# sandialabs/implicit-sph

Hardware: AMD Instinct MI355X
Metric: pressure-Poisson solves/sec (3D TGV, 1M particles per GPU, GMRES(50)+block-Jacobi ILU(0), tol 1e-8) (higher is better)
Workload: dtype f64; 1 GPU; 3D Taylor-Green vortex, 100^3 particles per GPU, Wendland cut=2h (BASELINE configs[1]), state after one Lagrangian step (mode=advect); rows_per_gpu=1000000, global_rows=1000000, nnz_per_gpu=103845090, solver=FGMRES(50) DGKS tol 1e-8, right prec, precond=bjacobi-ilu0, atom_order=lexicographic, library_row_order=bricks, parallelism=domain bricks 1x1x1, RCCL halo + all-reduce, restarts=1, converged=1

## Files before the change

### implicit-sph_amd/csrc/ilu.hpp

```cpp
#pragma once
#include <cfloat>
#include <cmath>
#include "core.hpp"
#include "sell.hpp"

struct isph_ilu {
  int n = 0, B = 0, nblocks = 0, wmax = 0;
  isph::DevBuf<long long> frp;
  isph::DevBuf<int> fcol, flen, fdiag, err;
  isph::DevBuf<double> fval;
  isph::DevBuf<double> sv;
  int value_bits = 64;
  isph::DevBuf<float> svf;
  isph::DevBuf<unsigned short> sc;
  isph::DevBuf<unsigned char> si;
  isph::DevBuf<unsigned short> sperm;
  isph::DevBuf<int> fdst;
  isph::DevBuf<int> blkinfo;
  isph::DevBuf<int> llev;
  isph::DevBuf<double> dinv;
  isph::DevBuf<long long> boff;
  isph::DevBuf<long long> sboff;
  bool exact = false;
  long long stream_entries = 0;
  bool compact = false;
  const long long *stream_off() const { return exact ? sboff.p : boff.p; }
  isph::DevBuf<unsigned char> flev;
  long long stream_chunks = 0;
  long long total = 0;
  int fill = 0;
  int capf = 0, slack = 0;
  isph::DevBuf<int> bptr;
  const int *blocks() const { return bptr.p; }
};

namespace isph {

__device__ __forceinline__ void ilu_block_rows(const int *__restrict__ bptr, int b, int B, int n, int &blo, int &bhi) {
  if (bptr) { blo = bptr[b]; bhi = bptr[b + 1]; }
  else { blo = b * B; bhi = min(blo + B, n); }
}

constexpr int kExtChunk = 8;
constexpr int kExtAhead = 8;

template <bool REFILL = false>
__global__ __launch_bounds__(1024) void k_ilu_extract(int n, int B, const int *__restrict__ rowlen,
                                                      const long long *__restrict__ slice_off,
                                                      const int *__restrict__ scol, const double *__restrict__ sval,
                                                      long long *__restrict__ frp, int *__restrict__ fcol,
                                                      double *__restrict__ fval, int *__restrict__ flen,
                                                      int *__restrict__ fdiag, int *__restrict__ err, int b0,
                                                      const long long *__restrict__ base_off,
                                                      const int *__restrict__ bptr, int *__restrict__ badrow = nullptr) {
  __shared__ int wsum[16];
  extern __shared__ double ext_lds[];
  const int nwv = blockDim.x >> 6;
  double (*stage_val)[64][kExtChunk] = reinterpret_cast<double (*)[64][kExtChunk]>(ext_lds);
  long long (*stage_start)[64] = reinterpret_cast<long long (*)[64]>(ext_lds + (size_t)nwv * 64 * kExtChunk);
  int (*stage_col)[64][kExtChunk] = reinterpret_cast<int (*)[64][kExtChunk]>(ext_lds + (size_t)nwv * 64 * (kExtChunk + 1));
  int (*stage_cnt)[64] = reinterpret_cast<int (*)[64]>(reinterpret_cast<int *>(ext_lds + (size_t)nwv * 64 * (kExtChunk + 1)) +
                                                       (size_t)nwv * 64 * kExtChunk);
  const int b = blockIdx.x + b0;
  int blo, bhi;
// ... 578 lines not shown
            sc[idx] = (unsigned short)flags;
            sv[idx] = 0.0;
          }
        }
        if (rinfo & 1) {
          const unsigned need = (unsigned)((rinfo >> 1) & 7);
          for (int c = lane; c < rT; c += 64) si[rch0 + c] = (unsigned char)((c == rT - 1 ? 1u : 0u) | (need << 1));
          const int first = (rinfo >> 8) & 127, nun = 64 - first;
          for (int x = lane; x < rT * nun; x += 64) {
            const int c = x / nun, ln = first + x - c * nun;
            const long long idx = (rch0 + c) * 64 + ln;
            sc[idx] = 0;
            sv[idx] = 0.0;
          }
        }
      };
      int cja = colreq(0), cjb;
      for (int src = 0; src < 64; src += 2) {
        cjb = colreq(src + 1);
        emit(src, cja);
        cja = colreq(src + 2);
        emit(src + 1, cjb);
      }
    }
    used += s_nch;
    __syncthreads();
  }
}

constexpr int kFacPrefetch = 4;
constexpr int kFacPrefetchWide = 8;
constexpr int kIluWaves = 8;

template <int WAVES, bool WIDE>
__global__ __launch_bounds__(WAVES * 64, WIDE ? 1 : 8) void k_ilu_factor(int n, int B, int W, const long long *__restrict__ frp,
                                                           const int *__restrict__ fcol, double *__restrict__ fval,
                                                           const int *__restrict__ flen,
                                                           const int *__restrict__ fdiag, const int *__restrict__ fdst,
                                                           const int *__restrict__ llev, double *__restrict__ sv,
                                                           double *__restrict__ dinv, const long long *__restrict__ boff,
                                                           int capf, int slack, int b0, const int *__restrict__ err,
                                                           const int *__restrict__ bptr) {
  extern __shared__ double lds_f[];
  double *diag = lds_f;
  double *wval = diag + B;
  long long *rpL = reinterpret_cast<long long *>(wval + WAVES * W);
  int *wcol = reinterpret_cast<int *>(rpL + B);
  int *lenL = wcol + WAVES * W;
  int *dgL = lenL + B;
  int *lstart = dgL + B;
  int *lcnt = lstart + B + 2;
  int *levs = lcnt + B + 1;
  unsigned short *order = reinterpret_cast<unsigned short *>(levs + B);
  unsigned short *pos = order + B;
  __shared__ int s_nlev, s_err;
  if (threadIdx.x == 0) s_err = err != nullptr ? *err : 0;
  __syncthreads();
  if (s_err & (1 | 16 | 32)) return;
  const int bid = blockIdx.x + b0;
  int blo, bhi;
  ilu_block_rows(bptr, bid, B, n, blo, bhi);
  const int m = bhi - blo;
  const int wave = threadIdx.x >> 6, lane = threadIdx.x & 63;
  double *svb = sv + ilu_base_chunk(boff, bid, capf, slack) * 64;
  if (threadIdx.x == 0) s_nlev = 0;
  for (int t = threadIdx.x; t <= B; t += blockDim.x) lcnt[t] = 0;
  for (int t = threadIdx.x; t < WAVES * B; t += blockDim.x) pos[t] = 0;
  __syncthreads();
  for (int t = threadIdx.x; t < m; t += blockDim.x) {
    rpL[t] = frp[blo + t];
    lenL[t] = flen[blo + t];
    dgL[t] = fdiag[blo + t];
    const int l = llev[blo + t];
    levs[t] = l;
    atomicAdd(&lcnt[l], 1);
    atomicMax(&s_nlev, l + 1);
  }
  __syncthreads();
  if (threadIdx.x == 0) {
    int run = 0;
    for (int l = 0; l < s_nlev; ++l) { lstart[l] = run; run += lcnt[l]; }
    lstart[s_nlev] = run;
  }
  __syncthreads();
  for (int t = threadIdx.x; t < m; t += blockDim.x) {
    const int l = levs[t];
    int rk = 0;
    for (int q = 0; q < t; ++q) rk += (levs[q] == l);
    order[lstart[l] + rk] = (unsigned short)t;
  }
  __syncthreads();
  double *mv = wval + wave * W;
  int *mc = wcol + wave * W;
  unsigned short *mp = pos + wave * B;
  const int nlev = s_nlev;
  const long long rp_block = (long long)(((unsigned long long)(unsigned)__builtin_amdgcn_readfirstlane((int)(rpL[0] >> 32)) << 32) |
                                         (unsigned)__builtin_amdgcn_readfirstlane((int)rpL[0]));
// ... 374 lines not shown
      if (hipGetLastError() != hipSuccess) rc = fail("ILU(k) symbolic fill failed", __FILE__, __LINE__);
    }
    if (rc != ISPH_SUCCESS) { nrp.release(); ncol.release(); ndiag.release(); nlev.release(); nval.release(); break; }
    F->frp.release(); F->fcol.release(); F->fdiag.release(); F->flev.release(); F->fval.release(); F->flen.release();
    F->frp = nrp; F->fcol = ncol; F->fdiag = ndiag; F->flev = nlev; F->fval = nval;
    F->flen = nlen;
    nlen = DevBuf<int>();
    rc = nlen.reserve(n1);
    F->total = total;
    F->wmax = wmax;
  }
  nlen.release(); inoff.release(); blktot.release(); meta.release();
  if (!ctx->pattern_hold || rc != ISPH_SUCCESS) F->flev.release();
  return rc;
}

inline long long &ilu_exact_stream_bytes() {
  static long long v = 4LL << 30;
  return v;
}
inline bool ilu_wants_exact_stream(const isph_ilu *F) {
  const long long rule_chunks = kCapFactor * (F->total >> 6) + (long long)(kPadChunks + 2 * F->B) * (F->nblocks + 1) + kPadChunks;
  return rule_chunks * 64 * 10 > ilu_exact_stream_bytes();
}
inline int ilu_size_stream(isph_ilu *F) {
  const long long entries = F->exact ? F->stream_entries : F->total;
  F->stream_chunks = F->capf * (entries >> 6) + (long long)(kPadChunks + F->slack) * (F->nblocks + 1) + kPadChunks;
  int r = F->sv.reserve((size_t)F->stream_chunks * 64);
  if (r == ISPH_SUCCESS) r = F->sc.reserve((size_t)F->stream_chunks * 64);
  if (r == ISPH_SUCCESS) r = F->si.reserve((size_t)F->stream_chunks + 64);
  return r;
}

inline int ilu_begin(isph_ctx *ctx, const Sell &S, int block_size, bool sgs, int fill, isph_ilu **out, bool defer_factor_arrays = false,
                     int nblocks_tab = 0, const int *host_bptr = nullptr) {
  ISPH_REQUIRE(block_size >= 64 && block_size <= 1024 && block_size % 64 == 0,
               "block-Jacobi ILU block size must be a multiple of 64 in [64,1024]");
  ISPH_REQUIRE(fill >= 0 && fill <= 8 && !(sgs && fill), "level of fill must be in [0,8]");
  ISPH_REQUIRE(nblocks_tab == 0 || host_bptr, "a table of subdomains without its offsets");
  isph_ilu *F = new isph_ilu();
  F->n = S.nrow; F->B = block_size; F->wmax = S.wmax; F->fill = fill;
  F->nblocks = nblocks_tab > 0 ? nblocks_tab : (S.nrow + block_size - 1) / block_size;
  if (nblocks_tab > 0) {
    if (F->bptr.reserve((size_t)nblocks_tab + 1) != ISPH_SUCCESS ||
        hipMemcpyAsync(F->bptr.p, host_bptr, sizeof(int) * ((size_t)nblocks_tab + 1), hipMemcpyHostToDevice, ctx->stream) != hipSuccess ||
        hipStreamSynchronize(ctx->stream) != hipSuccess) {
      ilu_destroy(F);
      return fail("copy of the subdomain table failed", __FILE__, __LINE__);
    }
  }
  F->total = S.stored + (nblocks_tab > 0 ? 64LL * nblocks_tab : 0);
  const size_t stored = (size_t)(F->total > 0 ? F->total : 1), n1 = (size_t)(S.nrow > 0 ? S.nrow : 1);
  F->capf = kCapFactor; F->slack = 2 * block_size;
  int rc = defer_factor_arrays ? ISPH_SUCCESS : F->fcol.reserve(stored);
  if (rc == ISPH_SUCCESS && !defer_factor_arrays) rc = F->fval.reserve(stored);
  if (rc == ISPH_SUCCESS) rc = F->frp.reserve(n1);
  if (rc == ISPH_SUCCESS) rc = F->flen.reserve(n1);
  if (rc == ISPH_SUCCESS) rc = F->fdiag.reserve(n1);
  if (rc == ISPH_SUCCESS) rc = F->dinv.reserve(n1);
  if (rc == ISPH_SUCCESS) rc = F->llev.reserve(n1);
  if (rc == ISPH_SUCCESS) rc = F->err.reserve(1);
  if (rc == ISPH_SUCCESS) rc = F->boff.reserve((size_t)F->nblocks + 1);
  if (rc == ISPH_SUCCESS) rc = F->blkinfo.reserve((size_t)4 * (F->nblocks > 0 ? F->nblocks : 1));
  if (rc == ISPH_SUCCESS) rc = F->sperm.reserve((size_t)2 * block_size * (F->nblocks > 0 ? F->nblocks : 1));
  if (rc == ISPH_SUCCESS && hipMemsetAsync(F->err.p, 0, sizeof(int), ctx->stream) != hipSuccess)
    rc = fail("memset failed", __FILE__, __LINE__);
  if (rc == ISPH_SUCCESS && S.nrow > 0) {
    const size_t lds_e = (size_t)(block_size / 64) * 64 * ((kExtChunk + 1) * 8 + (kExtChunk + 1) * 4);
    const size_t lds_s = sizeof(int) * (14 * (size_t)block_size + 10) + sizeof(long long) * (size_t)block_size;
    if (hipFuncSetAttribute(reinterpret_cast<const void *>(k_ilu_extract<false>), hipFuncAttributeMaxDynamicSharedMemorySize,
                            (int)lds_e) != hipSuccess ||
        hipFuncSetAttribute(reinterpret_cast<const void *>(k_ilu_schedule<true>), hipFuncAttributeMaxDynamicSharedMemorySize,
                            (int)lds_s) != hipSuccess ||
        hipFuncSetAttribute(reinterpret_cast<const void *>(k_ilu_schedule<false>), hipFuncAttributeMaxDynamicSharedMemorySize,
// ... 13 lines not shown
  return size_stream ? ilu_size_stream(F) : ISPH_SUCCESS;
}

inline void ilu_launch_extract(isph_ctx *ctx, isph_ilu *F, const Sell &S, int b0, int nb, hipStream_t st = nullptr) {
  const size_t lds_e = (size_t)(F->B / 64) * 64 * ((kExtChunk + 1) * 8 + (kExtChunk + 1) * 4);
  ProfScope prof(ctx, PROF_ILU_EXTRACT, st);
  hipLaunchKernelGGL(k_ilu_extract<false>, dim3(nb), dim3(F->B), lds_e, st ? st : ctx->stream, S.nrow, F->B, (const int *)S.rowlen.p,
                     (const long long *)S.slice_off.p, (const int *)S.col.p, (const double *)S.val.p, F->frp.p, F->fcol.p,
                     F->fval.p, F->flen.p, F->fdiag.p, F->err.p, b0, F->compact ? (const long long *)F->boff.p : (const long long *)nullptr,
                     F->blocks(), (int *)nullptr);
}

inline void ilu_launch_schedule(isph_ctx *ctx, isph_ilu *F, const Sell &S, int b0, int nb, bool sgs, hipStream_t st = nullptr,
                                bool count_only = false) {
  const size_t Bz = (size_t)F->B;
  const size_t lds_s = sizeof(int) * (14 * Bz + 10) + sizeof(long long) * Bz;
  ProfScope prof(ctx, PROF_ILU_SCHEDULE, st);
  if (F->wmax <= 129)
    hipLaunchKernelGGL(k_ilu_schedule<true>, dim3(nb), dim3(F->B), lds_s, st ? st : ctx->stream, S.nrow, F->B, F->stream_off(), F->frp.p, F->fcol.p,
                       F->flen.p, F->fdiag.p, F->sv.p, F->sc.p, F->si.p, F->sperm.p, F->fdst.p, F->blkinfo.p, F->llev.p, F->capf,
                       F->slack, F->err.p, sgs ? (const double *)F->fval.p : (const double *)nullptr,
                       sgs ? (const double *)F->dinv.p : (const double *)nullptr, b0, count_only ? 1 : 0, F->blocks());
  else
    hipLaunchKernelGGL(k_ilu_schedule<false>, dim3(nb), dim3(F->B), lds_s, st ? st : ctx->stream, S.nrow, F->B, F->stream_off(), F->frp.p, F->fcol.p,
                       F->flen.p, F->fdiag.p, F->sv.p, F->sc.p, F->si.p, F->sperm.p, F->fdst.p, F->blkinfo.p, F->llev.p, F->capf,
                       F->slack, F->err.p, sgs ? (const double *)F->fval.p : (const double *)nullptr,
                       sgs ? (const double *)F->dinv.p : (const double *)nullptr, b0, count_only ? 1 : 0, F->blocks());
}

inline int ilu_launch_factor(isph_ctx *ctx, isph_ilu *F, const Sell &S, int b0, int nb, const int *err_dev, hipStream_t st_in = nullptr) {
  hipStream_t st = st_in ? st_in : ctx->stream;
  const size_t Bz = (size_t)F->B;
  const int W = ((F->wmax + 63) / 64) * 64;
  const size_t lds_f = 8 * Bz + (size_t)kIluWaves * W * 12 + 8 * Bz + 4 * (5 * Bz + 4) + 2 * Bz + 2 * (size_t)kIluWaves * Bz + 16;
  ISPH_REQUIRE(lds_f <= 160 * 1024, "ILU factor kernel needs too much LDS for this row width");
  const bool wide = F->wmax > 128;
  const void *fk = wide ? reinterpret_cast<const void *>(k_ilu_factor<kIluWaves, true>)
                        : reinterpret_cast<const void *>(k_ilu_factor<kIluWaves, false>);
  ISPH_CHECK_HIP(hipFuncSetAttribute(fk, hipFuncAttributeMaxDynamicSharedMemorySize, (int)lds_f));
  ProfScope prof(ctx, PROF_ILU_FACTOR, st_in);
  if (wide)
    hipLaunchKernelGGL((k_ilu_factor<kIluWaves, true>), dim3(nb), dim3(kIluWaves * 64), lds_f, st, S.nrow, F->B, W,
                       F->frp.p, F->fcol.p, F->fval.p, F->flen.p, F->fdiag.p, F->fdst.p, F->llev.p, F->sv.p, F->dinv.p, F->stream_off(),
                       F->capf, F->slack, b0, err_dev, F->blocks());
  else
    hipLaunchKernelGGL((k_ilu_factor<kIluWaves, false>), dim3(nb), dim3(kIluWaves * 64), lds_f, st, S.nrow, F->B, W,
                       F->frp.p, F->fcol.p, F->fval.p, F->flen.p, F->fdiag.p, F->fdst.p, F->llev.p, F->sv.p, F->dinv.p, F->stream_off(),
                       F->capf, F->slack, b0, err_dev, F->blocks());
  ISPH_CHECK_HIP(hipGetLastError());
  return ISPH_SUCCESS;
}

inline int ilu_schedule_and_factor(isph_ctx *ctx, isph_ilu *F, const Sell &S, bool sgs) {
  int rc = ISPH_SUCCESS;
  if (sgs)
    hipLaunchKernelGGL(k_sgs_pivots, dim3((S.nrow + kBlock - 1) / kBlock), dim3(kBlock), 0, ctx->stream, S.nrow, F->frp.p,
                       F->fval.p, F->fdiag.p, F->dinv.p);
  if (F->exact) {
    rc = F->sboff.reserve((size_t)F->nblocks + 1);
    if (rc == ISPH_SUCCESS) {
      ilu_launch_schedule(ctx, F, S, 0, F->nblocks, sgs, nullptr, true);
      hipLaunchKernelGGL(k_ilu_exact_offsets, dim3(1), dim3(1024), 0, ctx->stream, F->nblocks, (const int *)F->blkinfo.p, F->sboff.p);
      long long total = 0;
      if (hipMemcpyAsync(&total, F->sboff.p + F->nblocks, sizeof(long long), hipMemcpyDeviceToHost, ctx->stream) != hipSuccess)
        rc = fail("copy failed", __FILE__, __LINE__);
      if (rc == ISPH_SUCCESS) rc = ilu_check_err(ctx, F, "ILU extract/schedule (counting pass) failed");
// ... 462 lines not shown
```

### implicit-sph_amd/csrc/isph_capi.hip

```cpp
#include <algorithm>
#include <numeric>

#include "assemble.hpp"
#include "operators.hpp"
#include "block_helmholtz.hpp"
#include "core.hpp"
#include "ilu.hpp"
#include "krylov.hpp"
#include "sell.hpp"
#include "solver.hpp"
#include "chebyshev.hpp"
#include "amg.hpp"
#include "schwarz.hpp"
#include "prec.hpp"
#include "gcrodr.hpp"
#include "ingress.hpp"

namespace isph {
thread_local std::string g_last_error;

int sell_finalize_offsets(isph_ctx *ctx, Sell &S) {
  hipLaunchKernelGGL(k_exclusive_scan_ll, dim3(1), dim3(1024), 0, ctx->stream, S.nslices, S.slice_off.p, S.slice_off.p);
  std::vector<long long> so((size_t)S.nslices + 1, 0);
  ISPH_CHECK_HIP(hipMemcpyAsync(so.data(), S.slice_off.p, sizeof(long long) * so.size(), hipMemcpyDeviceToHost, ctx->stream));
// ... 1112 lines not shown
  return type && parse_prec_type(type, &s) ? (int)s.kind : -1;
}

int isph_prec_value_bits(const isph_prec *M) {
  if (const Cheb *C = prec_cheb(M)) return C->value_bits;
  if (const isph_amg *G = prec_amg(M)) return G->cheb ? G->cheb_value_bits : 0;
  if (const isph_ilu *F = prec_ilu(M)) return F->value_bits == 32 ? 32 : 0;
  return 0;
}

int isph_prec_cycle_bits(const isph_prec *M) {
  const isph_amg *G = prec_amg(M);
  return (G && G->cheb && G->cycle_bits == 32) ? 32 : 64;
}

int isph_prec_create(isph_ctx *ctx, const isph_mat *A, const char *type, int block_size, isph_prec **Mout) {
  ISPH_REQUIRE(ctx && A && type && Mout, "NULL argument");
  return prec_create_named(ctx, A, type, block_size, Mout);
}

int isph_prec_refactor(isph_ctx *ctx, isph_prec *M, const isph_mat *A) {
  ISPH_REQUIRE(ctx && M && A, "NULL argument");
  return prec_refactor(ctx, M, A);
}

int isph_prec_apply(isph_ctx *ctx, const isph_prec *M, const double *r, double *z, int on_device) {
  ISPH_REQUIRE(ctx && M && r && z, "NULL argument");
  return prec_apply_operands(ctx, M, r, z, on_device);
}

int isph_prec_multi_path(isph_ctx *ctx, const isph_prec *M, int nvec) {
  if (!ctx || !M) return 0;
  return prec_multi_shared(M, nvec) ? 1 : 0;
}

int isph_prec_apply_multi(isph_ctx *ctx, const isph_prec *M, int nvec, const double *r, double *z, int lda, int on_device) {
  ISPH_REQUIRE(ctx && M && r && z, "NULL argument");
  ISPH_REQUIRE(nvec >= 1, "isph_prec_apply_multi: nvec must be at least 1");
  ISPH_REQUIRE(lda >= M->n, "isph_prec_apply_multi: lda must be at least the number of rows");
  return prec_apply_multi_operands(ctx, M, nvec, r, z, lda, on_device);
}

int isph_prec_export_ilu(isph_ctx *ctx, const isph_prec *M, int *rowptr, int *colidx, double *val) {
  ISPH_REQUIRE(ctx && prec_ilu(M), "not an ILU preconditioner");
  return ilu_export(ctx, M->ilu, rowptr, colidx, val);
}

int isph_prec_info(isph_ctx *ctx, const isph_prec *M, long long info[4]) {
  ISPH_REQUIRE(ctx && M && info, "NULL argument");
  info[0] = info[1] = info[2] = info[3] = 0;
  const isph_ilu *F = prec_ilu(M);
  if (!F) return ISPH_SUCCESS;
  std::vector<int> bi((size_t)4 * F->nblocks);
  ISPH_CHECK_HIP(hipMemcpyAsync(bi.data(), F->blkinfo.p, sizeof(int) * bi.size(), hipMemcpyDeviceToHost, ctx->stream));
  ISPH_CHECK_HIP(hipStreamSynchronize(ctx->stream));
  long long used = 0;
  for (size_t b = 0; b < (size_t)F->nblocks; ++b) used += bi[4 * b] + bi[4 * b + 1];
  info[0] = ilu_nnz(F); info[1] = used; info[2] = F->stream_chunks; info[3] = F->nblocks;
  return ISPH_SUCCESS;
}

long long isph_prec_nnz(const isph_prec *M) { return prec_ilu(M) ? ilu_nnz(M->ilu) : 0; }

void isph_prec_destroy(isph_prec *M) { prec_destroy(M); }


// ... 863 lines not shown
```

### implicit-sph_amd/hip.py

```python
import ctypes as C
import sys
import os

import numpy as np

from . import build as _build

UID_BYTES = 128
NOT_SINGULAR, NULLSPACE, PINZERO, DOUBLEDIAG = 0, 1, 2, 3
KERNELS = {"wendland": 0, "quintic": 1, "cubic": 2}

EXPORTS = [
    "isph_ctx_create", "isph_comm_unique_id", "isph_ctx_create_dist", "isph_ctx_create_hostcomm", "isph_ctx_sync", "isph_ctx_destroy", "isph_pool_trim", "isph_pool_set_cap", "isph_set_exact_stream_threshold", "isph_pool_cached_bytes", "isph_pool_info", "isph_halo_create", "isph_halo_forward", "isph_halo_destroy", "isph_prec_create_overlap",
    "isph_last_error", "isph_mat_create_csr", "isph_mat_create_csr_bjacobi", "isph_mat_create_csr_blocks", "isph_mat_create_csr_coords", "isph_mat_create_csr_coords_bjacobi", "isph_ingress_info", "isph_mat_set_halo", "isph_mat_info", "isph_mat_export_csr", "isph_mat_export_rows", "isph_mat_column_bits",
    "isph_mat_destroy", "isph_spmv", "isph_spmv_time", "isph_prec_create", "isph_prec_create_blocks", "isph_prec_create_blocks_fill", "isph_prec_apply",
    "isph_prec_apply_multi", "isph_prec_multi_path",
    "isph_prec_export_ilu", "isph_prec_nnz", "isph_prec_info", "isph_prec_destroy", "isph_solver_params_default", "isph_solve",
    "isph_ctx_set_profile", "isph_ctx_hold_neighbours", "isph_ctx_profile_read", "isph_ctx_set_ordering", "isph_ctx_set_periodic_box", "isph_mat_ordering_info", "isph_mat_ordering", "isph_mat_ordering_faces", "isph_ctx_halo_profile_read", "isph_ctx_comm_info", "isph_device_identity", "isph_assemble_poisson", "isph_assemble_helmholtz", "isph_assemble_solute_transport", "isph_assemble_applied_potential", "isph_compute_volumes", "isph_compute_pnd", "isph_compute_corrections", "isph_gradient", "isph_divergence", "isph_correct_velocity_pressure",
    "isph_advance_begin", "isph_advance_end", "isph_compute_shift", "isph_apply_shift", "isph_shift_particles",
    "isph_solve_block", "isph_assemble_block_helmholtz", "isph_amg_params_default", "isph_prec_create_amg", "isph_prec_amg_levels", "isph_prec_amg_info",
    "isph_prec_amg_export", "isph_prec_amg_aggregates", "isph_prec_amg_path", "isph_prec_amg_refreshes", "isph_prec_amg_set_nullvec",
    "isph_schwarz_params_default", "isph_prec_create_schwarz", "isph_prec_schwarz_info", "isph_prec_schwarz_paths", "isph_prec_schwarz_timing", "isph_prec_schwarz_export",
    "isph_pb_params_default", "isph_assemble_poisson_boltzmann", "isph_pb_residual", "isph_pb_jacobian", "isph_solve_poisson_boltzmann",
    "isph_compute_normals", "isph_csf_params_default", "isph_csf_phase_normal", "isph_csf_force", "isph_surface_tension_csf", "isph_pairwise_force",
    "isph_smooth_field", "isph_ek_params_default", "isph_electrostatic_force", "isph_random_stress_tensor", "isph_random_stress_force",
    "isph_force_from_random_stress", "isph_cheb_params_default", "isph_prec_create_chebyshev", "isph_prec_value_bits", "isph_prec_cycle_bits",
    "isph_prec_eig_estimate",
    "isph_poly_params_default", "isph_prec_create_gmres_poly", "isph_prec_poly_info", "isph_prec_type_kind",
    "isph_ilu_params_default", "isph_prec_create_ilu",
    "isph_nlist_build", "isph_nlist_info", "isph_nlist_get", "isph_nlist_destroy",
    "isph_nlist_build_dist", "isph_nlist_dist_info", "isph_nlist_dist_get", "isph_nlist_forward", "isph_nlist_forward_int",
    "isph_migrate", "isph_migrated_info", "isph_migrated_get", "isph_migrated_destroy",
    "isph_ctx_hold_pattern", "isph_mat_update_values", "isph_mat_pattern_info", "isph_prec_refactor",
    "isph_recycle_create", "isph_recycle_destroy", "isph_recycle_reset", "isph_recycle_info", "isph_recycle_export", "isph_recycle_import",
    "isph_solve_recycle", "isph_dense_tall_gemm", "isph_dense_block_gram",
    "isph_ghost_fill", "isph_zero_mean_pressure", "isph_status", "isph_tgv_error",
    "isph_ins_params_default", "isph_ins_create", "isph_ins_destroy", "isph_ins_set_state", "isph_ins_set_list", "isph_ins_rebuild",
    "isph_ins_sizes", "isph_ins_get", "isph_ins_pre", "isph_ins_view", "isph_ins_force", "isph_ins_add_force", "isph_ins_solve",
    "isph_ins_advance", "isph_ins_shift", "isph_ins_diagnostics", "isph_ins_run",
    "isph_nlist_forward_multi", "isph_zero_mean_pressure_dist", "isph_status_dist", "isph_tgv_error_dist",
    "isph_ins_create_dist", "isph_ins_set_state_dist", "isph_ins_sizes_dist",
]


class AmgParams(C.Structure):
    _fields_ = [("max_levels", C.c_int), ("coarse_max", C.c_int), ("omega", C.c_double), ("block", C.c_int),
                ("sweeps", C.c_int), ("theta", C.c_double), ("smoother", C.c_int), ("cheb_ratio", C.c_double),
                ("cheb_value_bits", C.c_int), ("eig_type", C.c_int), ("eig_iters", C.c_int), ("cycle_bits", C.c_int),
                ("ilu_fill", C.c_int)]
# ... 109 lines not shown
        L.isph_ctx_halo_profile_read.argtypes = [C.c_void_p, C.c_void_p, C.c_void_p]
        L.isph_ctx_comm_info.argtypes = [C.c_void_p, C.c_void_p]
        L.isph_device_identity.argtypes = [C.c_int, C.c_char_p]
        L.isph_ctx_set_ordering.argtypes = [C.c_void_p, C.c_int]
        L.isph_ctx_set_periodic_box.argtypes = [C.c_void_p, C.c_void_p, C.c_void_p, C.c_void_p]
        L.isph_mat_ordering_info.argtypes = [C.c_void_p, C.c_void_p, C.c_void_p]
        L.isph_mat_ordering.argtypes = [C.c_void_p, C.c_void_p, C.c_void_p, C.c_void_p]
        L.isph_mat_ordering_faces.argtypes = [C.c_void_p, C.c_int, C.c_void_p]
        L.isph_mat_create_csr.argtypes = [C.c_void_p, C.c_int, C.c_int, C.c_void_p, C.c_void_p, C.c_void_p,
                                          C.c_int, C.c_void_p]
        L.isph_mat_create_csr_bjacobi.argtypes = [C.c_void_p, C.c_int, C.c_int, C.c_void_p, C.c_void_p, C.c_void_p,
                                                  C.c_int, C.c_void_p, C.c_void_p]
        L.isph_mat_create_csr_blocks.argtypes = [C.c_void_p, C.c_int, C.c_int, C.c_void_p, C.c_void_p, C.c_void_p,
                                                 C.c_int, C.c_void_p, C.c_void_p, C.c_void_p]
        L.isph_mat_create_csr_coords.argtypes = [C.c_void_p, C.c_int, C.c_int, C.c_void_p, C.c_void_p, C.c_void_p, C.c_int,
                                                 C.c_void_p, C.c_void_p, C.c_void_p, C.c_void_p]
        L.isph_mat_create_csr_coords_bjacobi.argtypes = [C.c_void_p, C.c_int, C.c_int, C.c_void_p, C.c_void_p, C.c_void_p, C.c_int,
                                                         C.c_void_p, C.c_void_p, C.c_void_p, C.c_void_p, C.c_void_p]
        L.isph_mat_set_halo.argtypes = [C.c_void_p, C.c_void_p, C.c_int, C.c_void_p, C.c_void_p, C.c_void_p,
                                        C.c_void_p]
        L.isph_mat_info.argtypes = [C.c_void_p, C.c_void_p]
        L.isph_mat_export_csr.argtypes = [C.c_void_p, C.c_void_p, C.c_void_p, C.c_void_p, C.c_void_p]
        L.isph_mat_export_rows.argtypes = [C.c_void_p, C.c_void_p, C.c_int, C.c_int, C.c_void_p, C.c_void_p, C.c_void_p, C.c_longlong]
        L.isph_mat_column_bits.argtypes = [C.c_void_p, C.c_void_p, C.c_void_p]
        L.isph_mat_destroy.argtypes = [C.c_void_p]
        L.isph_spmv.argtypes = [C.c_void_p, C.c_void_p, C.c_void_p, C.c_void_p, C.c_int]
        L.isph_spmv_time.argtypes = [C.c_void_p, C.c_void_p, C.c_void_p, C.c_void_p, C.c_int, C.c_int, C.c_void_p]
        L.isph_prec_create.argtypes = [C.c_void_p, C.c_void_p, C.c_char_p, C.c_int, C.c_void_p]
        L.isph_prec_create_blocks.argtypes = [C.c_void_p, C.c_void_p, C.c_int, C.c_void_p, C.c_void_p]
        L.isph_prec_create_blocks_fill.argtypes = [C.c_void_p, C.c_void_p, C.c_int, C.c_void_p, C.c_int, C.c_void_p]
        L.isph_prec_apply.argtypes = [C.c_void_p, C.c_void_p, C.c_void_p, C.c_void_p, C.c_int]
        L.isph_prec_apply_multi.argtypes = [C.c_void_p, C.c_void_p, C.c_int, C.c_void_p, C.c_void_p, C.c_int, C.c_int]
        L.isph_prec_multi_path.argtypes = [C.c_void_p, C.c_void_p, C.c_int]
        L.isph_prec_export_ilu.argtypes = [C.c_void_p, C.c_void_p, C.c_void_p, C.c_void_p, C.c_void_p]
        L.isph_prec_destroy.argtypes = [C.c_void_p]
        L.isph_prec_info.argtypes = [C.c_void_p, C.c_void_p, C.c_void_p]
        L.isph_solve.argtypes = [C.c_void_p, C.c_void_p, C.c_void_p, C.c_void_p, C.c_void_p, C.c_int, C.c_int,
                                 C.c_int, C.c_void_p, C.c_void_p, C.c_void_p, C.c_int]
        L.isph_assemble_poisson.argtypes = [C.c_void_p, C.c_void_p, C.c_int, C.c_double, C.c_void_p, C.c_void_p,
                                            C.c_int, C.c_int, C.c_int, C.c_void_p, C.c_void_p, C.c_int]
        L.isph_compute_volumes.argtypes = [C.c_void_p, C.c_void_p, C.c_void_p, C.c_int]
        L.isph_compute_pnd.argtypes = [C.c_void_p, C.c_void_p, C.c_void_p, C.c_int]
        L.isph_compute_corrections.argtypes = [C.c_void_p, C.c_void_p, C.c_void_p, C.c_void_p, C.c_int]
        for fn in (L.isph_gradient, L.isph_divergence):
            fn.argtypes = [C.c_void_p, C.c_void_p, C.c_int, C.c_void_p, C.c_double, C.c_int, C.c_int, C.c_int,
                           C.c_void_p, C.c_int]
        L.isph_correct_velocity_pressure.argtypes = [C.c_void_p, C.c_void_p, C.c_int, C.c_double, C.c_void_p,
                                                     C.c_void_p, C.c_void_p, C.c_void_p, C.c_int, C.c_int]
        L.isph_advance_begin.argtypes = [C.c_void_p, C.c_void_p, C.c_int, C.c_double, C.c_void_p, C.c_void_p,
                                         C.c_void_p, C.c_void_p, C.c_int]
        L.isph_advance_end.argtypes = [C.c_void_p, C.c_int, C.c_int, C.c_double, C.c_void_p, C.c_void_p, C.c_void_p,
                                       C.c_void_p, C.c_void_p, C.c_int]
        L.isph_assemble_block_helmholtz.argtypes = [C.c_void_p, C.c_void_p, C.c_int, C.c_double, C.c_double, C.c_double,
                                                    C.c_void_p, C.c_void_p, C.c_void_p, C.c_void_p, C.c_void_p, C.c_int,
                                                    C.c_void_p, C.c_void_p, C.c_int, C.c_void_p, C.c_void_p, C.c_int,
                                                    C.c_int]
        L.isph_solve_block.argtypes = [C.c_void_p, C.c_int, C.c_void_p, C.c_void_p, C.c_void_p, C.c_void_p, C.c_int,
                                       C.c_void_p, C.c_void_p, C.c_int]
        L.isph_prec_create_schwarz.argtypes = [C.c_void_p, C.c_void_p, C.c_void_p, C.c_void_p]
        L.isph_prec_schwarz_info.argtypes = [C.c_void_p, C.c_void_p]
        L.isph_prec_schwarz_paths.argtypes = [C.c_void_p, C.c_void_p]
        L.isph_prec_schwarz_export.argtypes = [C.c_void_p] * 7
        L.isph_prec_schwarz_timing.argtypes = [C.c_void_p, C.c_void_p]
        L.isph_amg_params_default.argtypes = [C.c_void_p]
        L.isph_prec_create_amg.argtypes = [C.c_void_p, C.c_void_p, C.c_void_p, C.c_void_p, C.c_int, C.c_void_p]
        L.isph_prec_amg_levels.argtypes = [C.c_void_p]
# ... 540 lines not shown
        R = _f64(R)
        shape = tuple(R.shape)
        if len(shape) == 2:
            if nvec is None:
                nvec = shape[0]
            if lda is None:
                lda = shape[1]
        if nvec is None:
            raise OperandError("R is flat: nvec is needed")
        nvec, lda = int(nvec), int(self.n if lda is None else lda)
        if nvec < 1:
            raise OperandError("nvec = %d: at least one vector is needed" % nvec)
        if lda < self.n:
            raise OperandError("lda = %d is below the %d rows of the preconditioner" % (lda, self.n))
        if len(shape) == 2 and (shape[0] != nvec or shape[1] != lda):
            raise OperandError("R is %r, not [nvec = %d, lda = %d]" % (shape, nvec, lda))
        need = lda * (nvec - 1) + self.n
        _need(R, need, "R [lda x nvec]")
        if Z is None:
            if _is_torch(R):
                import torch
                Z = torch.zeros_like(R)
            else:
                Z = np.zeros_like(R)
        else:
            Z = _f64(Z)
        _need(Z, need, "Z [lda x nvec]")
        _check(lib().isph_prec_apply_multi(self.ctx.h, self.h, nvec, _ptr(R), _ptr(Z), lda, _on_device(R, Z)))
        return Z

    def multi_path(self, nvec):
        return int(lib().isph_prec_multi_path(self.ctx.h, self.h, int(nvec)))

    def refactor(self, A):
        _check(lib().isph_prec_refactor(self.ctx.h, self.h, A.h))
        if getattr(self, "A", None) is not None:
            self.A = A

    @property
    def value_bits(self):
        return int(lib().isph_prec_value_bits(self.h))

    @property
    def cycle_bits(self):
        return int(lib().isph_prec_cycle_bits(self.h))

    def eig_estimate(self, level=0):
        a = (C.c_double * 3)()
        _check(lib().isph_prec_eig_estimate(self.ctx.h, self.h, int(level), a))
        return dict(lambda_used=float(a[0]), rho=float(a[1]), steps=int(a[2]))

    def _poly_info(self):
        roots = np.zeros(2 * POLY_MAX_DEGREE)
        hess = np.zeros((POLY_MAX_DEGREE + 1) * POLY_MAX_DEGREE)
        deg = C.c_int()
        _check(lib().isph_prec_poly_info(self.h, _ptr(roots), _ptr(hess), C.byref(deg)))
        return roots, hess, deg.value

    def roots(self):
        roots, _, d = self._poly_info()
        return roots[0:2 * d:2] + 1j * roots[1:2 * d:2]

    def hessenberg(self):
        _, hess, d = self._poly_info()
        return hess.reshape(POLY_MAX_DEGREE, POLY_MAX_DEGREE + 1).T[:d + 1, :d].copy()

# ... 1397 lines not shown
```

### include/isph_hip.h

```cpp
#ifndef ISPH_HIP_H
#define ISPH_HIP_H

#ifdef __cplusplus
extern "C" {
#endif

typedef struct isph_ctx isph_ctx;
typedef struct isph_mat isph_mat;
typedef struct isph_prec isph_prec;

#define ISPH_SUCCESS 0
#define ISPH_FAILURE (-1)
#define ISPH_UID_BYTES 128


int isph_ctx_create(int device, void *stream, isph_ctx **ctx);
int isph_comm_unique_id(char *uid);
int isph_ctx_create_dist(int device, void *stream, int rank, int nranks,
                         const char *uid, isph_ctx **ctx);
typedef struct {
  void *user;
  int (*exchange)(void *user, int npeers, const int *peer, const double *send, const long long *send_off,
                  double *recv, const long long *recv_off);
  int (*allreduce)(void *user, double *buf, int count, int op);
// ... 79 lines not shown
int isph_prec_schwarz_export(isph_ctx *ctx, const isph_prec *M, int *rows, int *loc_ptr, long long *rowptr,
                             int *colidx, double *val);
int isph_prec_create_overlap(isph_ctx *ctx, const isph_mat *Aext, int nlocal, int level_of_fill, int combine, int npeers,
                             const int *peer_rank, const int *send_ptr, const int *send_idx, const int *recv_ptr,
                             isph_prec **M);

typedef struct {
  int degree;
  double ratio, lambda_max, lambda_min;
  int value_bits;
  int eig_type;
  int eig_iters;
} isph_cheb_params;
void isph_cheb_params_default(isph_cheb_params *p);
int isph_prec_create_chebyshev(isph_ctx *ctx, const isph_mat *A, const isph_cheb_params *prm, isph_prec **M);
int isph_prec_value_bits(const isph_prec *M);
int isph_prec_cycle_bits(const isph_prec *M);
int isph_prec_eig_estimate(isph_ctx *ctx, const isph_prec *M, int level, double out[3]);

typedef struct {
  int degree;
} isph_poly_params;
void isph_poly_params_default(isph_poly_params *p);
int isph_prec_create_gmres_poly(isph_ctx *ctx, const isph_mat *A, const isph_poly_params *prm,
                                const double *nullvec , int on_device, isph_prec **M);
int isph_prec_poly_info(const isph_prec *M, double *roots_re_im, double *hess, int *degree);
int isph_prec_type_kind(const char *type);

int isph_prec_apply(isph_ctx *ctx, const isph_prec *M, const double *r ,
                    double *z , int on_device);
int isph_prec_apply_multi(isph_ctx *ctx, const isph_prec *M, int nvec, const double *r ,
                          double *z , int lda, int on_device);
int isph_prec_multi_path(isph_ctx *ctx, const isph_prec *M, int nvec);
int isph_prec_export_ilu(isph_ctx *ctx, const isph_prec *M, int *rowptr, int *colidx, double *val);
long long isph_prec_nnz(const isph_prec *M);
int isph_prec_info(isph_ctx *ctx, const isph_prec *M, long long info[4]);
void isph_prec_destroy(isph_prec *M);


typedef struct {
  int solver_type;
  int flexible;
  int num_blocks;
  int max_iters;
  int max_restarts;
  double tol;
  int ortho;
  int verbose;
  int num_recycled;
  int basis_bits;
} isph_solver_params;
void isph_solver_params_default(isph_solver_params *p);

typedef struct {
  int converged, iters, restarts;
  double rel_res_implicit;
  double rel_res_explicit;
  double prec_setup_ms;
  double solve_ms;
  double spmv_ms;
  int spmv_calls;
  int reorth;
  int residual_restarts;
} isph_solve_info;

int isph_solve(isph_ctx *ctx, const isph_mat *A, const isph_prec *M,
// ... 348 lines not shown
```

Measured before the change: 25.38 solves/s (1M-particle bricks; x n_gpus under weak scaling).

## Add gather-based ILU(0) factorization kernel using LDS row bitmaps

Adds a new ILU(0) factor path. Each block builds per-row column bitmaps and popcount prefix tables in LDS, and each wave eliminates a row by gathering the needed upper-factor entries through bitmap lookup, with software prefetch and readlane broadcast of the multipliers. It replaces the scatter-based elimination for block sizes up to 512 and rows up to 128 wide. The aim is to cut LDS scatter traffic and synchronisation in the factorization, at the cost of more LDS per block and lower occupancy (launch bounds 6). An environment variable can force the old scatter path, and a new API call reports which path ran.

New measurement: 25.74 solves/s (1M-particle bricks; x n_gpus under weak scaling), median of 6. 1.4% higher.

```diff
diff --git a/implicit-sph_amd/csrc/ilu.hpp b/implicit-sph_amd/csrc/ilu.hpp
--- a/implicit-sph_amd/csrc/ilu.hpp
+++ b/implicit-sph_amd/csrc/ilu.hpp
@@ -1,6 +1,8 @@
 #pragma once
 #include <cfloat>
 #include <cmath>
+#include <cstdlib>
+#include <type_traits>
 #include "core.hpp"
 #include "sell.hpp"
 
@@ -30,6 +32,8 @@
   long long total = 0;
   int fill = 0;
   int capf = 0, slack = 0;
+  bool force_scatter = false;
+  int factor_path = 0;
   isph::DevBuf<int> bptr;
   const int *blocks() const { return bptr.p; }
 };
@@ -674,8 +678,263 @@
 constexpr int kFacPrefetchWide = 8;
 constexpr int kIluWaves = 8;
 
-template <int WAVES, bool WIDE>
-__global__ __launch_bounds__(WAVES * 64, WIDE ? 1 : 8) void k_ilu_factor(int n, int B, int W, const long long *__restrict__ frp,
+constexpr int kFacGatherPF = 4;
+
+__device__ __forceinline__ double ilu_readlane_f64(double v, int l) {
+  return __hiloint2double(__builtin_amdgcn_readlane(__double2hiint(v), l), __builtin_amdgcn_readlane(__double2loint(v), l));
+}
+
+struct IluGatherRow {
+  int r, len, dg;
+  unsigned rp;
+  int craw[2], dst[2];
+  double a[2];
+};
+
+template <int NS, int HP, int KPF>
+__device__ __forceinline__ void ilu_gather_steps(double (&a)[NS], const unsigned *const (&bml)[NS],
+                                                 const unsigned char *const (&pfl)[NS], const unsigned (&bit)[NS],
+                                                 const unsigned (&low)[NS], unsigned P, double pdv, int s_beg, int s_end,
+                                                 const char *fval_bytes) {
+  const int j_beg = s_beg - 64 * HP, nst = s_end - 64 * HP;
+  auto lookup = [&](int j, unsigned (&w)[NS], unsigned (&p)[NS], unsigned &ub8) {
+    const unsigned Pj = (unsigned)__builtin_amdgcn_readlane((int)P, j < nst ? j : j_beg);
+    const unsigned krow4 = Pj & 0x7fffu;
+    ub8 = (Pj >> 15) << 3;
+#pragma unroll
+    for (int h = 0; h < NS; ++h) {
+      w[h] = *reinterpret_cast<const unsigned *>(reinterpret_cast<const char *>(bml[h]) + krow4);
+      p[h] = pfl[h][krow4 >> 2];
+    }
+  };
+  auto request = [&](const unsigned (&w)[NS], const unsigned (&p)[NS], unsigned ub8, double (&u)[NS], bool (&mt)[NS]) {
+#pragma unroll
+    for (int h = 0; h < NS; ++h) {
+      mt[h] = (w[h] & bit[h]) != 0u;
+      const unsigned off = mt[h] ? ((((unsigned)__popc(w[h] & low[h]) + p[h]) << 3) + ub8) : 0u;
+      u[h] = *reinterpret_cast<const double *>(fval_bytes + off);
+    }
+  };
+  double uq[KPF][NS];
+  bool mq[KPF][NS];
+  unsigned w[NS], p[NS], w2[NS], p2[NS], ub8, ub8n;
+  lookup(j_beg, w, p, ub8);
+#pragma unroll
+  for (int u = 0; u < KPF; ++u) {
+    lookup(j_beg + u + 1, w2, p2, ub8n);
+    request(w, p, ub8, uq[u], mq[u]);
+#pragma unroll
+    for (int h = 0; h < NS; ++h) { w[h] = w2[h]; p[h] = p2[h]; }
+    ub8 = ub8n;
+    __builtin_amdgcn_sched_barrier(0);
+  }
+  for (int j0 = j_beg; j0 < nst; j0 += KPF) {
+#pragma unroll
+    for (int u = 0; u < KPF; ++u) {
+      const int j = j0 + u;
+      if (j < nst) {
+        const double lik = ilu_readlane_f64(a[HP] * pdv, j);
+#pragma unroll
+        for (int h = 0; h < NS; ++h)
+          if (mq[u][h]) a[h] -= lik * uq[u][h];
+      }
+      lookup(j + KPF + 1, w2, p2, ub8n);
+      request(w, p, ub8, uq[u], mq[u]);
+#pragma unroll
+      for (int h = 0; h < NS; ++h) { w[h] = w2[h]; p[h] = p2[h]; }
+      ub8 = ub8n;
+      __builtin_amdgcn_sched_barrier(0);
+    }
+  }
+}
+
+template <int KPF>
+__device__ __forceinline__ void ilu_gather_eliminate(IluGatherRow &R, int lane, int blo, int nw, const unsigned *bm,
+                                                     const unsigned char *pf, const unsigned *rpL, const unsigned short *dgL,
+                                                     const double *diag, const double *fval_b) {
+  const int dg = R.dg, len = R.len;
+  if (dg == 0) return;
+  const char *fval_bytes = reinterpret_cast<const char *>(fval_b);
+  const unsigned *bml[2];
+  const unsigned char *pfl[2];
+  unsigned bit[2], low[2], P[2];
+  double pd[2];
+#pragma unroll
+  for (int h = 0; h < 2; ++h) {
+    const int slot = lane + 64 * h;
+    const int cl = slot < len ? R.craw[h] - blo : 0;
+    bml[h] = bm + (cl >> 5);
+    pfl[h] = pf + (cl >> 5);
+    bit[h] = slot < len ? 1u << (cl & 31) : 0u;
+    low[h] = (1u << (cl & 31)) - 1u;
+    P[h] = 0u; pd[h] = 0.0;
+    if (slot < dg) {
+      P[h] = ((rpL[cl] + dgL[cl] + 1u) << 15) | (unsigned)(cl * nw * 4);
+      pd[h] = diag[cl];
+    }
+  }
+  if (dg > 64) {
+    ilu_gather_steps<2, 0, KPF>(R.a, bml, pfl, bit, low, P[0], pd[0], 0, 64, fval_bytes);
+    ilu_gather_steps<2, 1, KPF>(R.a, bml, pfl, bit, low, P[1], pd[1], 64, dg, fval_bytes);
+    if (lane + 64 < dg) R.a[1] *= pd[1];
+  } else {
+    const int nA = min(max(len - 64, 0), dg);
+    if (nA > 0) ilu_gather_steps<2, 0, KPF>(R.a, bml, pfl, bit, low, P[0], pd[0], 0, nA, fval_bytes);
+    if (nA < dg) {
+      const bool sel = lane < len - 64;
+      double am[1] = {sel ? R.a[1] : R.a[0]};
+      const unsigned *const bmm[1] = {sel ? bml[1] : bml[0]};
+      const unsigned char *const pfm[1] = {sel ? pfl[1] : pfl[0]};
+      const unsigned bitm[1] = {sel ? bit[1] : bit[0]}, lowm[1] = {sel ? low[1] : low[0]};
+      ilu_gather_steps<1, 0, KPF>(am, bmm, pfm, bitm, lowm, P[0], pd[0], nA, dg, fval_bytes);
+      if (sel) R.a[1] = am[0];
+      else R.a[0] = am[0];
+    }
+  }
+  if (lane < dg) R.a[0] *= pd[0];
+}
+
+template <int WAVES>
+__device__ __forceinline__ void ilu_factor_gather_block(double *lds, int B, int blo, int m, const long long *__restrict__ frp,
+                                                        const int *__restrict__ fcol, double *fval,
+                                                        const int *__restrict__ flen, const int *__restrict__ fdiag,
+                                                        const int *__restrict__ fdst, const int *__restrict__ llev,
+                                                        double *__restrict__ svb, double *__restrict__ dinv, int *s_nlev) {
+  const int nw = B >> 5;
+  double *diag = lds;
+  unsigned *rpL = reinterpret_cast<unsigned *>(diag + B);
+  unsigned *bm = rpL + B;
+  unsigned char *pf = reinterpret_cast<unsigned char *>(bm + B * nw);
+  int *lstart = reinterpret_cast<int *>(pf + B * nw);
+  unsigned short *lenL = reinterpret_cast<unsigned short *>(lstart + B + 2);
+  unsigned short *dgL = lenL + B;
+  unsigned short *order = dgL + B;
+  int *lcnt = reinterpret_cast<int *>(bm);
+  int *levs = lcnt + B + 1;
+  const int wave = __builtin_amdgcn_readfirstlane(threadIdx.x >> 6), lane = threadIdx.x & 63;
+  const long long rp_block = frp[blo];
+  const int *__restrict__ fcol_b = fcol + rp_block;
+  const int *__restrict__ fdst_b = fdst + rp_block;
+  double *fval_b = fval + rp_block;
+  if (threadIdx.x == 0) *s_nlev = 0;
+  for (int t = threadIdx.x; t <= B; t += blockDim.x) lcnt[t] = 0;
+  __syncthreads();
+  for (int t = threadIdx.x; t < m; t += blockDim.x) {
+    rpL[t] = (unsigned)(frp[blo + t] - rp_block);
+    lenL[t] = (unsigned short)flen[blo + t];
+    dgL[t] = (unsigned short)fdiag[blo + t];
+    const int l = llev[blo + t];
+    levs[t] = l;
+    atomicAdd(&lcnt[l], 1);
+    atomicMax(s_nlev, l + 1);
+  }
+  __syncthreads();
+  if (threadIdx.x == 0) {
+    int run = 0;
+    for (int l = 0; l < *s_nlev; ++l) { lstart[l] = run; run += lcnt[l]; }
+    lstart[*s_nlev] = run;
+  }
+  __syncthreads();
+  for (int t = threadIdx.x; t < m; t += blockDim.x) {
+    const int l = levs[t];
+    int rk = 0;
+    for (int q = 0; q < t; ++q) rk += (levs[q] == l);
+    order[lstart[l] + rk] = (unsigned short)t;
+  }
+  __syncthreads();
+  for (int t = threadIdx.x; t < B * nw; t += blockDim.x) bm[t] = 0u;
+  __syncthreads();
+  for (int t0 = wave; t0 < m; t0 += 8 * WAVES) {
+    int cq[8];
+#pragma unroll
+    for (int u = 0; u < 8; ++u) {
+      const int t = t0 + u * WAVES;
+      const int cnt = t < m ? (int)lenL[t] - (int)dgL[t] - 1 : 0;
+      const unsigned p = lane < cnt ? rpL[t] + dgL[t] + 1u + (unsigned)lane : 0u;
+      cq[u] = fcol_b[p];
+    }
+#pragma unroll
+    for (int u = 0; u < 8; ++u) {
+      const int t = t0 + u * WAVES;
+      const int cnt = t < m ? (int)lenL[t] - (int)dgL[t] - 1 : 0;
+      if (lane < cnt) {
+        const int c = cq[u] - blo;
+        atomicOr(&bm[t * nw + (c >> 5)], 1u << (c & 31));
+      }
+      for (int e = 64 + lane; e < cnt; e += 64) {
+        const int c = fcol_b[rpL[t] + dgL[t] + 1u + (unsigned)e] - blo;
+        atomicOr(&bm[t * nw + (c >> 5)], 1u << (c & 31));
+      }
+    }
+  }
+  __syncthreads();
+  for (int t = threadIdx.x; t < m; t += blockDim.x) {
+    unsigned run = 0;
+    for (int x = 0; x < nw; ++x) {
+      pf[t * nw + x] = (unsigned char)run;
+      run += (unsigned)__popc(bm[t * nw + x]);
+    }
+  }
+  __syncthreads();
+  const int nlev = *s_nlev;
+  int nl = 0, nq = wave;
+  auto settle = [&]() {
+    while (nl < nlev && nq >= __builtin_amdgcn_readfirstlane(lstart[nl + 1])) {
+      ++nl;
+      nq = __builtin_amdgcn_readfirstlane(lstart[nl]) + wave;
+    }
+  };
+  auto fetch = [&](IluGatherRow &R) {
+    const int r = __builtin_amdgcn_readfirstlane((int)order[nq]);
+    R.r = r;
+    R.rp = (unsigned)__builtin_amdgcn_readfirstlane((int)rpL[r]);
+    R.len = __builtin_amdgcn_readfirstlane((int)lenL[r]);
+    R.dg = __builtin_amdgcn_readfirstlane((int)dgL[r]);
+#pragma unroll
+    for (int h = 0; h < 2; ++h) {
+      R.craw[h] = 0; R.dst[h] = -1; R.a[h] = 0.0;
+      if (h == 0 || R.len > 64) {
+        const int slot = lane + 64 * h;
+        const unsigned p = R.rp + (unsigned)(slot < R.len ? slot : 0);
+        R.craw[h] = fcol_b[p];
+        R.a[h] = fval_b[p];
+        R.dst[h] = fdst_b[p];
+      }
+    }
+  };
+  IluGatherRow nx;
+  nx.r = 0; nx.len = 0; nx.dg = 0; nx.rp = 0;
+  nx.craw[0] = nx.craw[1] = 0; nx.dst[0] = nx.dst[1] = -1; nx.a[0] = nx.a[1] = 0.0;
+  settle();
+  if (nl < nlev) fetch(nx);
+  for (int l = 0; l < nlev; ++l) {
+    while (nl == l) {
+      IluGatherRow R = nx;
+      nq += WAVES;
+      settle();
+      if (nl < nlev) fetch(nx);
+      ilu_gather_eliminate<kFacGatherPF>(R, lane, blo, nw, bm, pf, rpL, dgL, diag, fval_b);
+#pragma unroll
+      for (int h = 0; h < 2; ++h) {
+        const int slot = lane + 64 * h;
+        if (slot < R.len) {
+          fval_b[R.rp + slot] = R.a[h];
+          if (R.dst[h] >= 0) svb[R.dst[h]] = R.a[h];
+        }
+      }
+      const double d = R.dg < 64 ? ilu_readlane_f64(R.a[0], R.dg) : ilu_readlane_f64(R.a[1], R.dg - 64);
+      if (lane == 0) {
+        const double rd = 1.0 / d;
+        diag[R.r] = rd;
+        dinv[blo + R.r] = rd;
+      }
+    }
+    __syncthreads();
+  }
+}
+
+template <int WAVES, bool WIDE, bool GATHER = false>
+__global__ __launch_bounds__(WAVES * 64, WIDE ? 1 : (GATHER ? 6 : 8)) void k_ilu_factor(int n, int B, int W, const long long *__restrict__ frp,
                                                            const int *__restrict__ fcol, double *__restrict__ fval,
                                                            const int *__restrict__ flen,
                                                            const int *__restrict__ fdiag, const int *__restrict__ fdst,
@@ -705,6 +964,10 @@
   const int m = bhi - blo;
   const int wave = threadIdx.x >> 6, lane = threadIdx.x & 63;
   double *svb = sv + ilu_base_chunk(boff, bid, capf, slack) * 64;
+  if constexpr (GATHER) {
+    ilu_factor_gather_block<WAVES>(lds_f, B, blo, m, frp, fcol, fval, flen, fdiag, fdst, llev, svb, dinv, &s_nlev);
+    return;
+  }
   if (threadIdx.x == 0) s_nlev = 0;
   for (int t = threadIdx.x; t <= B; t += blockDim.x) lcnt[t] = 0;
   for (int t = threadIdx.x; t < WAVES * B; t += blockDim.x) pos[t] = 0;
@@ -1145,6 +1408,12 @@
   return r;
 }
 
+inline bool ilu_factor_takes_gather(int B, int wmax) { return B <= 512 && wmax <= 128; }
+inline bool ilu_factor_scatter_forced() {
+  const char *env = getenv("ISPH_ILU_FACTOR_SCATTER");
+  return env && env[0] == '1';
+}
+
 inline int ilu_begin(isph_ctx *ctx, const Sell &S, int block_size, bool sgs, int fill, isph_ilu **out, bool defer_factor_arrays = false,
                      int nblocks_tab = 0, const int *host_bptr = nullptr) {
   ISPH_REQUIRE(block_size >= 64 && block_size <= 1024 && block_size % 64 == 0,
@@ -1153,6 +1422,7 @@
   ISPH_REQUIRE(nblocks_tab == 0 || host_bptr, "a table of subdomains without its offsets");
   isph_ilu *F = new isph_ilu();
   F->n = S.nrow; F->B = block_size; F->wmax = S.wmax; F->fill = fill;
+  F->force_scatter = ilu_factor_scatter_forced();
   F->nblocks = nblocks_tab > 0 ? nblocks_tab : (S.nrow + block_size - 1) / block_size;
   if (nblocks_tab > 0) {
     if (F->bptr.reserve((size_t)nblocks_tab + 1) != ISPH_SUCCESS ||
@@ -1232,6 +1502,19 @@
   hipStream_t st = st_in ? st_in : ctx->stream;
   const size_t Bz = (size_t)F->B;
   const int W = ((F->wmax + 63) / 64) * 64;
+  const bool gather = !F->force_scatter && ilu_factor_takes_gather(F->B, F->wmax);
+  F->factor_path = gather ? 1 : 0;
+  if (gather) {
+    const size_t lds_g = 8 * Bz + 4 * Bz + 5 * Bz * Bz / 32 + 4 * (Bz + 2) + 6 * Bz;
+    const void *gk = reinterpret_cast<const void *>(k_ilu_factor<kIluWaves, false, true>);
+    ISPH_CHECK_HIP(hipFuncSetAttribute(gk, hipFuncAttributeMaxDynamicSharedMemorySize, (int)lds_g));
+    ProfScope prof(ctx, PROF_ILU_FACTOR, st_in);
+    hipLaunchKernelGGL((k_ilu_factor<kIluWaves, false, true>), dim3(nb), dim3(kIluWaves * 64), lds_g, st, S.nrow, F->B, W,
+                       F->frp.p, F->fcol.p, F->fval.p, F->flen.p, F->fdiag.p, F->fdst.p, F->llev.p, F->sv.p, F->dinv.p, F->stream_off(),
+                       F->capf, F->slack, b0, err_dev, F->blocks());
+    ISPH_CHECK_HIP(hipGetLastError());
+    return ISPH_SUCCESS;
+  }
   const size_t lds_f = 8 * Bz + (size_t)kIluWaves * W * 12 + 8 * Bz + 4 * (5 * Bz + 4) + 2 * Bz + 2 * (size_t)kIluWaves * Bz + 16;
   ISPH_REQUIRE(lds_f <= 160 * 1024, "ILU factor kernel needs too much LDS for this row width");
   const bool wide = F->wmax > 128;
diff --git a/implicit-sph_amd/csrc/isph_capi.hip b/implicit-sph_amd/csrc/isph_capi.hip
--- a/implicit-sph_amd/csrc/isph_capi.hip
+++ b/implicit-sph_amd/csrc/isph_capi.hip
@@ -1168,6 +1168,12 @@
 int isph_prec_multi_path(isph_ctx *ctx, const isph_prec *M, int nvec) {
   if (!ctx || !M) return 0;
   return prec_multi_shared(M, nvec) ? 1 : 0;
+}
+
+int isph_prec_ilu_factor_path(isph_ctx *ctx, const isph_prec *M) {
+  if (!ctx || !M) return 0;
+  const isph_ilu *F = prec_ilu(M);
+  return F ? F->factor_path : 0;
 }
 
 int isph_prec_apply_multi(isph_ctx *ctx, const isph_prec *M, int nvec, const double *r, double *z, int lda, int on_device) {
diff --git a/implicit-sph_amd/hip.py b/implicit-sph_amd/hip.py
--- a/implicit-sph_amd/hip.py
+++ b/implicit-sph_amd/hip.py
@@ -14,7 +14,7 @@
     "isph_ctx_create", "isph_comm_unique_id", "isph_ctx_create_dist", "isph_ctx_create_hostcomm", "isph_ctx_sync", "isph_ctx_destroy", "isph_pool_trim", "isph_pool_set_cap", "isph_set_exact_stream_threshold", "isph_pool_cached_bytes", "isph_pool_info", "isph_halo_create", "isph_halo_forward", "isph_halo_destroy", "isph_prec_create_overlap",
     "isph_last_error", "isph_mat_create_csr", "isph_mat_create_csr_bjacobi", "isph_mat_create_csr_blocks", "isph_mat_create_csr_coords", "isph_mat_create_csr_coords_bjacobi", "isph_ingress_info", "isph_mat_set_halo", "isph_mat_info", "isph_mat_export_csr", "isph_mat_export_rows", "isph_mat_column_bits",
     "isph_mat_destroy", "isph_spmv", "isph_spmv_time", "isph_prec_create", "isph_prec_create_blocks", "isph_prec_create_blocks_fill", "isph_prec_apply",
-    "isph_prec_apply_multi", "isph_prec_multi_path",
+    "isph_prec_apply_multi", "isph_prec_multi_path", "isph_prec_ilu_factor_path",
     "isph_prec_export_ilu", "isph_prec_nnz", "isph_prec_info", "isph_prec_destroy", "isph_solver_params_default", "isph_solve",
     "isph_ctx_set_profile", "isph_ctx_hold_neighbours", "isph_ctx_profile_read", "isph_ctx_set_ordering", "isph_ctx_set_periodic_box", "isph_mat_ordering_info", "isph_mat_ordering", "isph_mat_ordering_faces", "isph_ctx_halo_profile_read", "isph_ctx_comm_info", "isph_device_identity", "isph_assemble_poisson", "isph_assemble_helmholtz", "isph_assemble_solute_transport", "isph_assemble_applied_potential", "isph_compute_volumes", "isph_compute_pnd", "isph_compute_corrections", "isph_gradient", "isph_divergence", "isph_correct_velocity_pressure",
     "isph_advance_begin", "isph_advance_end", "isph_compute_shift", "isph_apply_shift", "isph_shift_particles",
@@ -190,6 +190,7 @@
         L.isph_prec_apply.argtypes = [C.c_void_p, C.c_void_p, C.c_void_p, C.c_void_p, C.c_int]
         L.isph_prec_apply_multi.argtypes = [C.c_void_p, C.c_void_p, C.c_int, C.c_void_p, C.c_void_p, C.c_int, C.c_int]
         L.isph_prec_multi_path.argtypes = [C.c_void_p, C.c_void_p, C.c_int]
+        L.isph_prec_ilu_factor_path.argtypes = [C.c_void_p, C.c_void_p]
         L.isph_prec_export_ilu.argtypes = [C.c_void_p, C.c_void_p, C.c_void_p, C.c_void_p, C.c_void_p]
         L.isph_prec_destroy.argtypes = [C.c_void_p]
         L.isph_prec_info.argtypes = [C.c_void_p, C.c_void_p, C.c_void_p]
@@ -796,6 +797,9 @@
     def multi_path(self, nvec):
         return int(lib().isph_prec_multi_path(self.ctx.h, self.h, int(nvec)))
 
+    def factor_path(self):
+        return int(lib().isph_prec_ilu_factor_path(self.ctx.h, self.h))
+
     def refactor(self, A):
         _check(lib().isph_prec_refactor(self.ctx.h, self.h, A.h))
         if getattr(self, "A", None) is not None:
diff --git a/include/isph_hip.h b/include/isph_hip.h
--- a/include/isph_hip.h
+++ b/include/isph_hip.h
@@ -135,6 +135,7 @@
 int isph_prec_apply_multi(isph_ctx *ctx, const isph_prec *M, int nvec, const double *r ,
                           double *z , int lda, int on_device);
 int isph_prec_multi_path(isph_ctx *ctx, const isph_prec *M, int nvec);
+int isph_prec_ilu_factor_path(isph_ctx *ctx, const isph_prec *M);
 int isph_prec_export_ilu(isph_ctx *ctx, const isph_prec *M, int *rowptr, int *colidx, double *val);
 long long isph_prec_nnz(const isph_prec *M);
 int isph_prec_info(isph_ctx *ctx, const isph_prec *M, long long info[4]);
```
